# cassiePython/NeRF-Art

Measured on AMD Instinct MI355X. Metric: rays/sec at 480x270x128spp VolSDF render, higher is better.
Workload: dtype pixels bf16x3 (sdf, nabla, radiance, compositing of the 192 final samples: f32 split into 2 bf16 terms, 3 MFMAs per product, f32 accumulate), Algorithm-1 sampler fp16x1 on error-compensated one-term weights (fp16 act x fp16 weight, 1 MFMA per product, f32 accumulate; model.calibrate_sampler()), guar

## Files before the change

include/nerfart_hip.h:

```cpp
#ifndef NERFART_HIP_H
#define NERFART_HIP_H

#include <stddef.h>

#ifdef __cplusplus
extern "C" {
#endif

int nerfart_abi_version(void);
const char* nerfart_last_error(void);

int nerfart_profile_begin(void);
int nerfart_profile_end(double* ms, long long* launches, long long* units);
int nerfart_profile_end5(double* ms, long long* launches, long long* units);

void nerfart_linspace(float start, float end, int n, float* out);

int nerfart_sdf_fwd(const float* surf_blob, int precision, const float* pts, long long M, float R_bg, float* sdf_out, void* stream);
int nerfart_sdf_fwd_rays(const float* surf_blob, int precision, const float* rays_o, const float* rays_d, const int* ray_idx,
                         const float* depth, int n_slots, int n_per_ray, int depth_stride, float R_bg,
                         float* sdf_out, int out_stride, void* stream);

long long nerfart_sdf_nabla_workspace_bytes(int precision);
int nerfart_sdf_nabla_fwd(const float* surf_blob, int precision, const float* pts, long long M, float R_bg, float* sdf_out,
// ... 20 lines not shown
int nerfart_sdf_bwd2(const float* surf_blob, long long M, const float* gbar_h7, const float* gbar_sdf, void* f2_dump, void* r2_dump,
                     void* stream);

int nerfart_get_rays(const float* pose_dev, const float* K_dev, int H, int W, const long long* select_dev, int n,
                     float* rays_o, float* rays_d, void* stream);
int nerfart_normalize_dirs(const float* in, float* out, int n, void* stream);
int nerfart_linspace_depths(const float* t_dev, int n, const float* near, const float* far, float near_s, float far_s,
                            int n_rays, float* out, int stride, void* stream);

int nerfart_volsdf_first_check(int n_rays, int n, int cap, int n_final, float eps, float alpha_net, float beta_net,
                               const float* dA, const float* sA, const float* u_final, int u_final_stride,
                               float beta_plus0_denom, const float* far, float far_s, float* d_fine, float* beta_plus,
                               float* beta_map, float* iter_usage, int* act_out, int* act_count, void* stream);
int nerfart_volsdf_upsample(int n_active, int n, int cap, int n_up, const float* dA, const float* sA, const int* act,
                            const float* beta_plus, const float* u_up, int clamp_bounds, float* d_new, void* stream);
int nerfart_volsdf_merge_check(int n_active, int n, int cap, int n_up, int n_final, int max_bisect, int it, float eps,
                               float alpha_net, float beta_net, const float* dA, const float* sA, float* dB, float* sB,
                               const int* act, const float* d_new, const float* s_new, const float* u_final,
                               int u_final_stride, float* d_fine, float* beta_plus, float* beta_map, float* iter_usage,
                               int* act_out, int* act_count, void* stream);
int nerfart_volsdf_finalize(int n_active, int n, int cap, int n_final, const float* dA, const float* sA, const int* act,
                            const float* u_final, int u_final_stride, const float* beta_plus, float* d_fine,
                            float* beta_map, float* iter_usage, void* stream);
long long nerfart_volsdf_sampler_workspace_bytes(int n_rays, int n_init, int n_up, int n_final, int max_iter);
int nerfart_volsdf_fine_sample(const float* surf_blob, int precision, const float* rays_o, const float* rays_dn, int n_rays,
                               const float* near, const float* far, float near_s, float far_s, float R_bg,
                               float alpha_net, float beta_net, float eps, int n_init, int n_up, int n_final,
                               int max_iter, int max_bisect, const float* t_init_dev, const float* u_up_dev,
                               const float* u_final_dev, int u_final_per_ray, float* d_fine, float* beta_map,
                               float* iter_usage, void* workspace, long long workspace_bytes, void* stream);


int nerfart_volsdf_fine_sample_guarded(const float* surf_blob, int precision, const float* esc_blob, int esc_precision, float guard,
                                       const float* rays_o, const float* rays_dn, int n_rays,
                                       const float* near, const float* far, float near_s, float far_s, float R_bg,
                                       float alpha_net, float beta_net, float eps, int n_init, int n_up, int n_final,
                                       int max_iter, int max_bisect, const float* t_init_dev, const float* u_up_dev,
                                       const float* u_final_dev, int u_final_per_ray, float* d_fine, float* beta_map,
                                       float* iter_usage, int* n_escalated, void* workspace, long long workspace_bytes, void* stream);

int nerfart_volsdf_fine_sample_guarded2(const float* surf_blob, int precision, const float* esc_blob, int esc_precision, float guard, int late_round,
                                        const float* rays_o, const float* rays_dn, int n_rays,
                                        const float* near, const float* far, float near_s, float far_s, float R_bg,
                                        float alpha_net, float beta_net, float eps, int n_init, int n_up, int n_final,
                                        int max_iter, int max_bisect, const float* t_init_dev, const float* u_up_dev,
                                        const float* u_final_dev, int u_final_per_ray, float* d_fine, float* beta_map,
// ... 246 lines not shown
```

nerfart_amd/csrc/ray_common.h:

```cpp
#pragma once
#include "nerfart_common.h"
#include "sample_cdf.h"
#include <math.h>

namespace nerfart {

__device__ __forceinline__ float wave_sum(float v) {
#pragma unroll
    for (int o = 32; o > 0; o >>= 1) v += __shfl_xor(v, o, 64);
    return v;
}
__device__ __forceinline__ float wave_max(float v) {
#pragma unroll
    for (int o = 32; o > 0; o >>= 1) v = fmaxf(v, __shfl_xor(v, o, 64));
    return v;
}
__device__ __forceinline__ float wave_excl_sum(float v) {
    const int lane = threadIdx.x & 63;
#pragma unroll
    for (int o = 1; o < 64; o <<= 1) {
        const float t = __shfl_up(v, o, 64);
        if (lane >= o) v += t;
    }
    const float e = __shfl_up(v, 1, 64);
// ... 141 lines not shown
            const float sg = sdf_to_sigma(C.s[i], alpha, beta);
            const float t = a4b * C.dd[i];
            const float x = expf(-C.dstar[i] / beta);
            c_sigma[i] = sg; c_t[i] = t; c_x[i] = x;
            sR = __fmaf_rn(C.delta[i], sg, sR);
            sE = __fmaf_rn(t, x, sE);
        }
    }
    float R = wave_excl_sum(sR), E = wave_excl_sum(sE);
    float mx = -INFINITY;
#pragma unroll
    for (int i = 0; i < MAXSEG; ++i) {
        if (i < C.cnt) {
            E = __fmaf_rn(c_t[i], c_x[i], E);
            float b = expf(-R) * (expf(E) - 1.f);
            if (isnan(b)) b = INFINITY;
            mx = fmaxf(mx, b);
            R = __fmaf_rn(C.delta[i], c_sigma[i], R);
        }
    }
    return wave_max(mx);
}

__device__ __forceinline__ float error_bound_scan(const float* d, const float* s, int n, float alpha, float beta,
                                                  float* w_out, bool clamp) {
#ifndef NERFART_SCAN_GENERIC
    const int seg = (n - 1 + 63) >> 6;
    if (seg <= 8) return error_bound_scan_cached<8>(d, s, n, alpha, beta, w_out, clamp);
    if (seg <= 16) return error_bound_scan_cached<16>(d, s, n, alpha, beta, w_out, clamp);
    if (seg <= 24) return error_bound_scan_cached<24>(d, s, n, alpha, beta, w_out, clamp);
#endif
    return error_bound_scan_generic(d, s, n, alpha, beta, w_out, clamp);
}

__device__ __forceinline__ void opacity_cdf(const float* d, const float* s, int n, float alpha, float beta, float* cdf) {
    const int lane = threadIdx.x & 63;
    const int nint = n - 1;
    const int seg = (nint + 63) >> 6;
    const int k0 = lane * seg;
    const int k1 = (k0 + seg < nint) ? k0 + seg : nint;
    float sR = 0.f;
    for (int k = k0; k < k1; ++k) sR += sdf_to_sigma(s[k], alpha, beta) * (d[k + 1] - d[k]);
    float R = wave_excl_sum(sR);
    if (lane == 0) cdf[0] = 0.f;
    for (int k = k0; k < k1; ++k) {
        cdf[k + 1] = 1.f - expf(-R);
// ... 24 lines not shown
```

nerfart_amd/csrc/volsdf_render.hip:

```cpp
#include "ray_common.h"
#include "host_util.h"
#include <cstdlib>

namespace nerfart {

struct SamplerParams {
    int n;
    int cap;
    int n_up;
    int n_final;
    int max_bisect;
    int it;
    float eps;
    float alpha_net, beta_net;
    int u_final_stride;
    float guard;
    int* esc_list;
    int* esc_count;
};

__device__ __forceinline__ bool in_guard_band(const SamplerParams& P, float mx) {
    return P.guard > 0.f && fabsf(mx - P.eps) <= P.guard * P.eps;
}
__device__ __forceinline__ void escalate(const SamplerParams& P, int ray) {
    if (threadIdx.x == 0) P.esc_list[atomicAdd(P.esc_count, 1)] = ray;
}

__global__ void k_linspace_depths(const float* __restrict__ t, int n, const float* __restrict__ near,
                                  const float* __restrict__ far, float near_s, float far_s, int n_rays,
                                  float* __restrict__ out, int stride) {
    const long long i = (long long)blockIdx.x * blockDim.x + threadIdx.x;
    if (i >= (long long)n_rays * n) return;
    const int r = (int)(i / n), k = (int)(i - (long long)r * n);
    const float nr = near ? near[r] : near_s, fr = far ? far[r] : far_s;
    const float tk = t[k];
    out[(size_t)r * stride + k] = __fadd_rn(__fmul_rn(nr, __fsub_rn(1.f, tk)), __fmul_rn(fr, tk));
}

__global__ void k_normalize_dirs(const float* __restrict__ in, float* __restrict__ out, int n) {
    const int i = blockIdx.x * blockDim.x + threadIdx.x;
    if (i >= n) return;
// ... 68 lines not shown
}

template <int MAXSEG>
__device__ __forceinline__ void merge_check_tail(const SamplerParams& P, int ray, const float* d, const float* s, float* cdf, int nm,
                                                 const float* __restrict__ u_final, float* __restrict__ d_fine, float* __restrict__ beta_plus,
                                                 float* __restrict__ beta_map, float* __restrict__ iter_usage, int* __restrict__ act_out,
                                                 int* __restrict__ act_count) {
    constexpr int NS = MAXSEG > 0 ? MAXSEG : 1;
    SegConsts<NS> C;
    if constexpr (MAXSEG > 0) load_seg_consts<NS>(d, s, nm, C);
    auto scan = [&](float alpha, float beta) -> float {
        if constexpr (MAXSEG > 0) return scan_consts<NS>(C, alpha, beta);
        else return error_bound_scan(d, s, nm, alpha, beta, nullptr, false);
    };
    const float mx = scan(P.alpha_net, P.beta_net);
    if (in_guard_band(P, mx)) { escalate(P, ray); return; }
    if (!(mx > P.eps)) {
        opacity_cdf(d, s, nm, P.alpha_net, P.beta_net, cdf);
        __syncthreads();
        emit_final_samples(d, cdf, nm, u_final + (size_t)ray * P.u_final_stride, P.n_final, d_fine + (size_t)ray * P.n_final);
        if (threadIdx.x == 0) { iter_usage[ray] = (float)P.it; beta_map[ray] = P.beta_net; }
    } else {
        float hi = beta_plus[ray], lo = P.beta_net;
        for (int b = 0; b < P.max_bisect; ++b) {
            const float mid = 0.5f * (lo + hi);
            const float m = scan(1.f / mid, mid);
            if (m <= P.eps) hi = mid; else lo = mid;
        }
        if (threadIdx.x == 0) {
            beta_plus[ray] = hi;
            act_out[atomicAdd(act_count, 1)] = ray;
        }
    }
}

__global__ void __launch_bounds__(64)
k_merge_check(SamplerParams P, const float* __restrict__ dA, const float* __restrict__ sA,
              float* __restrict__ dB, float* __restrict__ sB, const int* __restrict__ act,
              const float* __restrict__ d_new, const float* __restrict__ s_new, const float* __restrict__ u_final,
              float* __restrict__ d_fine, float* __restrict__ beta_plus, float* __restrict__ beta_map,
              float* __restrict__ iter_usage, int* __restrict__ act_out, int* __restrict__ act_count) {
    extern __shared__ __attribute__((aligned(16))) float sm[];
    const int slot = blockIdx.x, ray = act[slot];
    const int n = P.n, nu = P.n_up, nm = n + nu;
    float* d_old = sm; float* dn = sm + n;
    float* d = dn + nu; float* s = d + nm;
    const float* s_old = sA + (size_t)ray * P.cap;
    const float* sn = s_new + (size_t)slot * nu;
    load_row(d_old, dA + (size_t)ray * P.cap, n);
    load_row(dn, d_new + (size_t)slot * nu, nu);
    __syncthreads();
    for (int i = threadIdx.x; i < n; i += 64) {
        const int r = i + lower_bound(dn, nu, d_old[i]);
        d[r] = d_old[i]; s[r] = s_old[i];
// ... 189 lines not shown
    const int first = blockIdx.x * 1024;
    int part = 0;
    for (int i = t; i < first; i += 1024) part += alive[i];
#pragma unroll
    for (int o = 32; o > 0; o >>= 1) part += __shfl_xor(part, o, 64);
    if (lane == 0) wsum[wv] = part;
    __syncthreads();
    if (t == 0) { int b = 0; for (int w = 0; w < 16; ++w) b += wsum[w]; base_sh = b; }
    __syncthreads();
    const int base = base_sh;
    const int slot = first + t;
    const bool keep = slot < n_live && alive[slot] != 0;
    const unsigned long long mask = __ballot(keep);
    const int rank = __popcll(mask & ((1ull << lane) - 1ull));
    __syncthreads();
    if (lane == 0) wsum[wv] = __popcll(mask);
    __syncthreads();
    int before = 0, total = 0;
    for (int w = 0; w < 16; ++w) { const int c = wsum[w]; if (w < wv) before += c; total += c; }
    if (keep) live_next[base + before + rank] = live[slot];
    if (t == 0 && first + 1024 >= n_live) *n_next = base + total;
}

}

using namespace nerfart;

extern "C" {

void nerfart_linspace(float start, float end, int n, float* out) {
    if (n == 1) { out[0] = start; return; }
    const float step = (end - start) / (float)(n - 1);
    const int half = n / 2;
    for (int i = 0; i < n; ++i) out[i] = (i < half) ? start + step * (float)i : end - step * (float)(n - i - 1);
}

int nerfart_normalize_dirs(const float* in, float* out, int n, void* stream) {
    if (n <= 0) return 0;
    hipLaunchKernelGGL(k_normalize_dirs, dim3((n + 255) / 256), dim3(256), 0, (hipStream_t)stream, in, out, n);
    NERFART_HIP(hipGetLastError());
    return 0;
}

int nerfart_linspace_depths(const float* t_dev, int n, const float* near, const float* far, float near_s, float far_s,
                            int n_rays, float* out, int stride, void* stream) {
    const long long tot = (long long)n_rays * n;
// ... 46 lines not shown
    if (n_up & (n_up - 1)) { set_last_error("n_up must be a power of two"); return 2; }
    SamplerParams P{n, cap, n_up, 0, 0, 0, 0.f, 0.f, 0.f};
    const size_t lds = ((size_t)4 * n + n_up) * sizeof(float);
    if (int rc = set_lds((const void*)k_upsample, lds, kLdsRefusal)) return rc;
    const char* e = std::getenv("NERFART_UPSAMPLE_SORT");
    const int always_sort = (e != nullptr && e[0] == 'a') ? 1 : 0;
    hipLaunchKernelGGL(k_upsample, dim3(n_active), dim3(64), lds, (hipStream_t)stream, P, dA, sA, act, beta_plus, u_up,
                       clamp_bounds, always_sort, d_new);
    NERFART_HIP(hipGetLastError());
    return 0;
}

int nerfart_volsdf_upsample(int n_active, int n, int cap, int n_up, const float* dA, const float* sA, const int* act,
                            const float* beta_plus, const float* u_up, int clamp_bounds, float* d_new, void* stream) {
    if (n_active <= 0) return 0;
    if (int rc = check_rows("volsdf_upsample", n, cap, 0)) return rc;
    return upsample_launch(n_active, n, cap, n_up, dA, sA, act, beta_plus, u_up, clamp_bounds, d_new, stream);
}

static int merge_check_launch(int n_active, int n, int cap, int n_up, int n_final, int max_bisect, int it, float eps,
                              float alpha_net, float beta_net, const float* dA, const float* sA, float* dB, float* sB,
                              const int* act, const float* d_new, const float* s_new, const float* u_final,
                              int u_final_stride, float* d_fine, float* beta_plus, float* beta_map, float* iter_usage,
                              int* act_out, int* act_count, float guard, int* esc_list, int* esc_count, void* stream) {
    if (n_active <= 0) return 0;
    SamplerParams P{n, cap, n_up, n_final, max_bisect, it, eps, alpha_net, beta_net, u_final_stride, guard, esc_list, esc_count};
    const size_t lds = ((size_t)3 * n + 3 * n_up) * sizeof(float);
    if (int rc = set_lds((const void*)k_merge_check, lds, kLdsRefusal)) return rc;
    hipLaunchKernelGGL(k_merge_check, dim3(n_active), dim3(64), lds, (hipStream_t)stream, P, dA, sA, dB, sB, act, d_new,
                       s_new, u_final, d_fine, beta_plus, beta_map, iter_usage, act_out, act_count);
    NERFART_HIP(hipGetLastError());
    return 0;
}

int nerfart_volsdf_merge_check(int n_active, int n, int cap, int n_up, int n_final, int max_bisect, int it, float eps,
                               float alpha_net, float beta_net, const float* dA, const float* sA, float* dB, float* sB,
                               const int* act, const float* d_new, const float* s_new, const float* u_final,
                               int u_final_stride, float* d_fine, float* beta_plus, float* beta_map, float* iter_usage,
                               int* act_out, int* act_count, void* stream) {
    if (n_active <= 0) return 0;
    if (int rc = check_rows("volsdf_merge_check", n, cap, n_up)) return rc;
    return merge_check_launch(n_active, n, cap, n_up, n_final, max_bisect, it, eps, alpha_net, beta_net, dA, sA, dB, sB, act, d_new, s_new, u_final,
                              u_final_stride, d_fine, beta_plus, beta_map, iter_usage, act_out, act_count, 0.f, nullptr, nullptr, stream);
}

static int finalize_launch(int n_active, int n, int cap, int n_final, const float* dA, const float* sA, const int* act,
                           const float* u_final, int u_final_stride, const float* beta_plus, float* d_fine,
                           float* beta_map, float* iter_usage, void* stream) {
    if (n_active <= 0) return 0;
    SamplerParams P{n, cap, 0, n_final, 0, 0, 0.f, 0.f, 0.f, u_final_stride};
    const size_t lds = (size_t)3 * n * sizeof(float);
    if (int rc = set_lds((const void*)k_finalize_unconverged, lds, kLdsRefusal)) return rc;
    hipLaunchKernelGGL(k_finalize_unconverged, dim3(n_active), dim3(64), lds, (hipStream_t)stream, P, dA, sA, act,
                       u_final, beta_plus, d_fine, beta_map, iter_usage);
    NERFART_HIP(hipGetLastError());
    return 0;
}

int nerfart_volsdf_finalize(int n_active, int n, int cap, int n_final, const float* dA, const float* sA, const int* act,
                            const float* u_final, int u_final_stride, const float* beta_plus, float* d_fine,
                            float* beta_map, float* iter_usage, void* stream) {
    if (n_active <= 0) return 0;
    if (int rc = check_rows("volsdf_finalize", n, cap, 0)) return rc;
    return finalize_launch(n_active, n, cap, n_final, dA, sA, act, u_final, u_final_stride, beta_plus, d_fine, beta_map, iter_usage, stream);
}

// ... 9 lines not shown
    return 0;
}

int nerfart_volsdf_composite(int n_rays, int P, const float* d_all, const float* sdf, const float* radiance,
                             const float* nabla, float alpha, float beta, int white_bkgd, float* rgb, float* depth,
                             float* acc, float* normals, float* sigma_out, float* p_out, float* tau_out, void* stream) {
    if (n_rays <= 0) return 0;
    if (P < 2) { set_last_error("volsdf_composite: needs P >= 2 samples per ray (P - 1 intervals)"); return 2; }
    if (normals && !nabla) { set_last_error("composite: normals requested without nablas"); return 2; }
    hipLaunchKernelGGL(k_composite_volsdf, dim3(n_rays), dim3(64), 0, (hipStream_t)stream, P, d_all, sdf, radiance, nabla,
                       alpha, beta, white_bkgd, rgb, depth, acc, normals, sigma_out, p_out, tau_out);
    NERFART_HIP(hipGetLastError());
    return 0;
}

typedef struct {
    float *dA, *sA, *dB, *sB, *d_new, *s_new, *beta_plus;
    int *act0, *act1, *count;
    float *t_init, *u_up, *u_final;
    int* esc_list;
    float *c_o, *c_dn, *c_near, *c_far, *c_u, *c_d_fine, *c_beta, *c_iter;
} sampler_ws_t;

enum { COUNT_SLOTS = 64, ESC_SLOT = COUNT_SLOTS - 1 };

static sampler_ws_t carve_sampler(Carver& c, int R, int cap, int n_up, int n0, int n_final) {
    sampler_ws_t w;
    const size_t row = (size_t)R * cap;
    w.dA = c.take<float>(row);
    w.sA = c.take<float>(row);
    w.dB = c.take<float>(row);
    w.sB = c.take<float>(row);
    w.d_new = c.take<float>((size_t)R * n_up);
    w.s_new = c.take<float>((size_t)R * n_up);
    w.beta_plus = c.take<float>((size_t)R);
    w.act0 = c.take<int>((size_t)R);
    w.act1 = c.take<int>((size_t)R);
    w.count = c.take<int>(COUNT_SLOTS);
    w.t_init = c.take<float>((size_t)n0);
    w.u_up = c.take<float>((size_t)(n_up + 2));
    w.u_final = c.take<float>((size_t)n_final);
    w.esc_list = c.take<int>((size_t)R);
    w.c_o = c.take<float>((size_t)R * 3);
    w.c_dn = c.take<float>((size_t)R * 3);
    w.c_near = c.take<float>((size_t)R);
    w.c_far = c.take<float>((size_t)R);
    w.c_u = c.take<float>((size_t)R * n_final);
// ... 3 lines not shown
    return w;
}

static size_t sampler_bytes(int R, int cap, int n_up, int n0, int n_final) {
    Carver c(nullptr);
    carve_sampler(c, R, cap, n_up, n0, n_final);
    return c.off;
}

long long nerfart_volsdf_sampler_workspace_bytes(int n_rays, int n_init, int n_up, int n_final, int max_iter) {
    return (long long)sampler_bytes(n_rays, n_init + max_iter * n_up, n_up, n_init, n_final);
}

static int fine_sample_run(const float* surf_blob, int precision, const float* esc_blob, int esc_precision, float guard, int late_round,
                           const float* rays_o, const float* rays_dn, int n_rays,
                           const float* near, const float* far, float near_s, float far_s, float R_bg,
                           float alpha_net, float beta_net, float eps, int n_init, int n_up, int n_final,
                           int max_iter, int max_bisect, const float* t_init_dev, const float* u_up_dev,
                           const float* u_final_dev, int u_final_per_ray, float* d_fine, float* beta_map,
                           float* iter_usage, void* workspace, long long workspace_bytes, int* n_escalated, hipStream_t stream) {
    if (n_escalated) *n_escalated = 0;
    if (n_rays <= 0) return 0;
    if (u_final_per_ray && !u_final_dev) { set_last_error("fine_sample: u_final_per_ray needs u_final_dev [n_rays, n_final]"); return 2; }
    if (max_iter < 0 || max_iter >= ESC_SLOT) { set_last_error("fine_sample: max_iter must be in [0, 62]"); return 2; }
    const bool guarded = esc_blob != nullptr && guard > 0.f;
    if (!guarded) guard = 0.f;
    const int u_stride = u_final_per_ray ? n_final : 0;
    const int cap = n_init + max_iter * n_up;
    Carver carver(workspace);
    sampler_ws_t w = carve_sampler(carver, n_rays, cap, n_up, n_init, n_final);
    if (!workspace || (size_t)workspace_bytes < carver.off) { set_last_error("fine_sample: workspace too small"); return 2; }
    const bool own_tables = !(t_init_dev && u_up_dev && u_final_dev);
    if (!own_tables) {
        w.t_init = const_cast<float*>(t_init_dev); w.u_up = const_cast<float*>(u_up_dev); w.u_final = const_cast<float*>(u_final_dev);
    } else {
        if (int rc = upload_linspace_tables({{w.t_init, n_init}, {w.u_up, n_up + 2}, {w.u_final, n_final}}, stream)) return rc;
        if (u_final_per_ray) w.u_final = const_cast<float*>(u_final_dev);
    }
    if (int rc = nerfart_linspace_depths(w.t_init, n_init, near, far, near_s, far_s, n_rays, w.dA, cap, stream)) return rc;
    if (int rc = nerfart_sdf_fwd_rays(surf_blob, precision, rays_o, rays_dn, nullptr, w.dA, n_rays, n_init, cap, R_bg, w.sA, cap, stream)) return rc;
    NERFART_HIP(hipMemsetAsync(w.count, 0, COUNT_SLOTS * sizeof(int), stream));
    const float denom = (float)(4.0 * (double)(n_init - 1) * log(1.0 + (double)eps));
    if (int rc = first_check_launch(n_rays, n_init, cap, n_final, eps, alpha_net, beta_net, w.dA, w.sA, w.u_final,
                                    u_stride, denom, far, far_s, d_fine, w.beta_plus, beta_map, iter_usage, w.act0,
                                    w.count, guard, w.esc_list, w.count + ESC_SLOT, stream)) return rc;
    int h_count[COUNT_SLOTS];
    NERFART_HIP(hipMemcpyAsync(h_count, w.count, sizeof(h_count), hipMemcpyDeviceToHost, stream));
    NERFART_HIP(hipStreamSynchronize(stream));
    int n_act = h_count[0];
    float *dA = w.dA, *sA = w.sA, *dB = w.dB, *sB = w.sB;
    int *act = w.act0, *act_next = w.act1;
    int n = n_init;
    for (int it = 1; it <= max_iter && n_act > 0; ++it) {
        if (int rc = upsample_launch(n_act, n, cap, n_up, dA, sA, act, w.beta_plus, w.u_up, it > 1, w.d_new, stream)) return rc;
        if (int rc = nerfart_sdf_fwd_rays(surf_blob, precision, rays_o, rays_dn, act, w.d_new, n_act, n_up, n_up, R_bg, w.s_new, n_up, stream)) return rc;
        if (int rc = merge_check_launch(n_act, n, cap, n_up, n_final, max_bisect, it, eps, alpha_net, beta_net, dA, sA,
                                        dB, sB, act, w.d_new, w.s_new, w.u_final, u_stride, d_fine, w.beta_plus,
                                        beta_map, iter_usage, act_next, w.count + it, guard, w.esc_list, w.count + ESC_SLOT, stream)) return rc;
        NERFART_HIP(hipMemcpyAsync(h_count, w.count, sizeof(h_count), hipMemcpyDeviceToHost, stream));
        NERFART_HIP(hipStreamSynchronize(stream));
        n_act = h_count[it];
        float* t;
        t = dA; dA = dB; dB = t;
        t = sA; sA = sB; sB = t;
        int* ti = act; act = act_next; act_next = ti;
        n += n_up;
        if (guarded && late_round > 0 && it >= late_round) break;
    }
    if (!guarded) {
        if (n_act > 0)
            if (int rc = finalize_launch(n_act, n, cap, n_final, dA, sA, act, w.u_final, u_stride, w.beta_plus, d_fine,
                                         beta_map, iter_usage, stream)) return rc;
        return 0;
    }
    int n_esc = h_count[ESC_SLOT];
    if (n_act > 0) {
        NERFART_HIP(hipMemcpyAsync(w.esc_list + n_esc, act, sizeof(int) * (size_t)n_act, hipMemcpyDeviceToDevice, stream));
        n_esc += n_act;
    }
    if (n_escalated) *n_escalated = n_esc;
    if (n_esc == 0) return 0;
    hipLaunchKernelGGL(k_gather_rays, dim3(n_esc), dim3(64), 0, stream, w.esc_list, n_esc, rays_o, rays_dn, near, far,
                       u_final_per_ray ? u_final_dev : (const float*)nullptr, n_final, w.c_o, w.c_dn, w.c_near, w.c_far, w.c_u);
    NERFART_HIP(hipGetLastError());
    const float* u2 = u_final_per_ray ? w.c_u : (own_tables ? nullptr : u_final_dev);
    const int* esc_list = w.esc_list;
    float *c_d_fine = w.c_d_fine, *c_beta = w.c_beta, *c_iter = w.c_iter;
    profile_class0_as(4);
    const int rc_esc = fine_sample_run(esc_blob, esc_precision, nullptr, 0, 0.f, 0, w.c_o, w.c_dn, n_esc, near ? w.c_near : nullptr, far ? w.c_far : nullptr,
                                       near_s, far_s, R_bg, alpha_net, beta_net, eps, n_init, n_up, n_final, max_iter, max_bisect,
                                       own_tables ? nullptr : t_init_dev, own_tables ? nullptr : u_up_dev, u2, u_final_per_ray, c_d_fine, c_beta, c_iter,
// ... 254 lines not shown
```

nerfart_amd/hip.py:

```python
from __future__ import annotations

import ctypes as C
import os

import torch

_HERE = os.path.dirname(os.path.abspath(__file__))
LIB_PATH = os.environ.get("NERFART_HIP_LIB", os.path.join(_HERE, "csrc", "libnerfart_hip.so"))

if not os.path.exists(LIB_PATH):
    raise ImportError(
        f"{LIB_PATH} not found: build the gfx950 kernels first "
        f"(python -c 'import __graft_entry__ as g; g.build()'  or  python -m nerfart_amd.build). "
        f"nerfart_amd has no CPU / eager-PyTorch fallback.")

lib = C.CDLL(LIB_PATH)


def csrc_sha256() -> str:
    import glob
    import hashlib
    h = hashlib.sha256()
    for f in sorted(glob.glob(os.path.join(_HERE, "csrc", "*.hip")) + glob.glob(os.path.join(_HERE, "csrc", "*.h"))
                    + glob.glob(os.path.join(_HERE, "csrc", "*.cpp"))):
# ... 11 lines not shown
    "nerfart_profile_end5": (_i, [_p, _p, _p]),
    "nerfart_sdf_fwd": (_i, [_p, _i, _p, _ll, _f, _p, _p]),
    "nerfart_sdf_fwd_rays": (_i, [_p, _i, _p, _p, _p, _p, _i, _i, _i, _f, _p, _i, _p]),
    "nerfart_sdf_nabla_workspace_bytes": (_ll, [_i]),
    "nerfart_sdf_nabla_fwd": (_i, [_p, _i, _p, _ll, _f, _p, _p, _p, _p, _ll, _p]),
    "nerfart_sdf_nabla_fwd_rays": (_i, [_p, _i, _p, _p, _p, _p, _i, _i, _i, _f, _p, _p, _p, _p, _ll, _p]),
    "nerfart_wgrad_workspace_bytes": (_ll, [_i, _ll, _i]),
    "nerfart_wgrad_bf16": (_i, [_p, _ll, _p, _ll, _i, _ll, _i, _ll, _p, _p, _i, _p, _ll, _p]),
    "nerfart_ray_points": (_i, [_p, _p, _p, _ll, _i, _p, _p, _p]),
    "nerfart_volsdf_pass2_cotangents": (_i, [_p, _p, _p, _p, _p, _p, _ll, _i, _f, _f, _ll, _p, _p, _p, _p]),
    "nerfart_wgrad_operand_embed_pair": (_i, [_p, _p, _ll, _ll, _i, _p, _p]),
    "nerfart_wgrad_operand_inputs": (_i, [_p, _i, _p, _i, _p, _ll, _ll, _p, _p]),
    "nerfart_wgrad_operand_rgb_delta": (_i, [_p, _p, _ll, _ll, _p, _p, _p, _p]),
    "nerfart_wgrad_operand_sbar_ones": (_i, [_p, _ll, _ll, _p, _p]),
    "nerfart_radiance_fwd": (_i, [_p, _i, _i, _p, _p, _ll, _p, _p, _p, _p]),
    "nerfart_radiance_fwd_rays": (_i, [_p, _i, _i, _p, _p, _p, _p, _i, _i, _i, _p, _p, _p, _p]),
    "nerfart_get_rays": (_i, [_p, _p, _i, _i, _p, _i, _p, _p, _p]),
    "nerfart_normalize_dirs": (_i, [_p, _p, _i, _p]),
    "nerfart_linspace_depths": (_i, [_p, _i, _p, _p, _f, _f, _i, _p, _i, _p]),
    "nerfart_volsdf_first_check": (_i, [_i, _i, _i, _i, _f, _f, _f, _p, _p, _p, _i, _f, _p, _f, _p, _p, _p, _p, _p, _p, _p]),
    "nerfart_volsdf_upsample": (_i, [_i, _i, _i, _i, _p, _p, _p, _p, _p, _i, _p, _p]),
    "nerfart_volsdf_merge_check": (_i, [_i, _i, _i, _i, _i, _i, _i, _f, _f, _f] + [_p] * 8 + [_i] + [_p] * 7),
    "nerfart_volsdf_finalize": (_i, [_i, _i, _i, _i] + [_p] * 4 + [_i] + [_p] * 5),
    "nerfart_volsdf_sampler_workspace_bytes": (_ll, [_i, _i, _i, _i, _i]),
    "nerfart_volsdf_fine_sample": (_i, [_p, _i, _p, _p, _i, _p, _p, _f, _f, _f, _f, _f, _f, _i, _i, _i, _i, _i, _p, _p, _p, _i, _p, _p, _p, _p, _ll, _p]),
    "nerfart_volsdf_fine_sample_guarded": (_i, [_p, _i, _p, _i, _f, _p, _p, _i, _p, _p, _f, _f, _f, _f, _f, _f, _i, _i, _i, _i, _i, _p, _p, _p, _i, _p, _p, _p, _p, _p, _ll, _p]),
    "nerfart_volsdf_fine_sample_guarded2": (_i, [_p, _i, _p, _i, _f, _i, _p, _p, _i, _p, _p, _f, _f, _f, _f, _f, _f, _i, _i, _i, _i, _i, _p, _p, _p, _i, _p, _p, _p, _p, _p, _ll, _p]),
    "nerfart_sort_concat": (_i, [_i, _p, _i, _i, _p, _i, _i, _p, _i, _p]),
    "nerfart_volsdf_composite": (_i, [_i, _i, _p, _p, _p, _p, _f, _f, _i] + [_p] * 8),
    "nerfart_volsdf_composite_bwd": (_i, [_i, _i, _p, _p, _p, _f, _f, _i, _p, _p, _p, _p, _p, _p]),
    "nerfart_neus_composite_bwd": (_i, [_i, _i, _p, _p, _f, _i, _p, _p, _p, _p, _p, _p]),
    "nerfart_volsdf_composite_geo_bwd": (_i, [_i, _i, _p, _p, _p, _f, _f, _p, _p, _p, _i, _p, _p, _p, _p]),
    "nerfart_sdf_fwd2_dump_bytes": (_ll, [_ll]),
    "nerfart_sdf_bwd2_dump_bytes": (_ll, [_ll]),
    "nerfart_sdf_fwd2": (_i, [_p, _p, _p, _ll, _p, _p]),
    "nerfart_sdf_bwd2": (_i, [_p, _ll, _p, _p, _p, _p, _p]),
    "nerfart_radiance_dump_bytes": (_ll, [_ll]),
    "nerfart_radiance_fwd_dump": (_i, [_p, _i, _p, _p, _ll, _p, _p, _p, _p, _p]),
    "nerfart_radiance_bwd": (_i, [_p, _ll, _p, _p, _p, _p, _p, _p, _p]),
    "nerfart_volsdf_render_workspace_bytes": (_ll, [_i, _i, _i, _i, _i]),
    "nerfart_volsdf_render_fwd": (_i, [_p, _p, _i, _i, _p, _p, _i, _f, _f, _f, _f, _f, _f, _i, _i, _i, _i, _i, _i] + [_p] * 4 + [_i] + [_p] * 13 + [_p, _ll, _p]),
    "nerfart_volsdf_render_mixed_fwd": (_i, [_p, _p, _i, _p, _i, _i, _p, _p, _i, _f, _f, _f, _f, _f, _f, _i, _i, _i, _i, _i, _i] + [_p] * 4 + [_i] + [_p] * 13 + [_p, _ll, _p]),
    "nerfart_volsdf_render_staged_fwd": (_i, [_p, _i, _p, _i, _p, _i, _f, _i, _p, _p, _i, _f, _f, _f, _f, _f, _f, _i, _i, _i, _i, _i, _i] + [_p] * 4 + [_i] + [_p] * 13 + [_p, _p, _ll, _p]),
    "nerfart_volsdf_render_staged2_fwd": (_i, [_p, _i, _p, _i, _p, _i, _f, _i, _i, _p, _p, _i, _f, _f, _f, _f, _f, _f, _i, _i, _i, _i, _i, _i] + [_p] * 4 + [_i] + [_p] * 13 + [_p, _p, _ll, _p]),
    "nerfart_near_far_from_sphere": (_i, [_p, _p, _i, _f, _p, _p, _p]),
    "nerfart_neus_upsample_step": (_i, [_i, _i, _i, _i, _f, _p, _p, _p, _i, _p, _p]),
# ... 703 lines not shown
    key = (n, str(device))
    if key not in _lin_cache:
        _lin_cache[key] = torch.linspace(0, 1, n).float().to(device)
    return _lin_cache[key]


_ws_cache = {}
_ws_lock = __import__("threading").Lock()


def _workspace(nbytes: int, device) -> torch.Tensor:
    key = (str(device), int(torch.cuda.current_stream(device).cuda_stream))
    with _ws_lock:
        ws = _ws_cache.get(key)
        if ws is None or ws.numel() < nbytes:
            _ws_cache.pop(key, None)
            while len(_ws_cache) >= 8:
                _ws_cache.pop(next(iter(_ws_cache)), None)
            ws = torch.empty(int(nbytes), dtype=torch.uint8, device=device)
            _ws_cache[key] = ws
    return ws


def volsdf_fine_sample(surf_blob, rays_o, rays_dn, near: float, far: float, R_bg: float, alpha: float, beta: float,
                       eps: float, n_init: int, n_up: int, n_final: int, max_iter: int, max_bisect: int, precision: int = 0,
                       u_final=None, escalate=None, guard: float = 0.0, stats=None, late_round: int = 0):
    R = rays_o.shape[0]
    dev = rays_o.device
    if u_final is not None and tuple(u_final.shape) != (R, n_final):
        raise ValueError(f"u_final must be [{R}, {n_final}]")
    d_fine = torch.empty(R, n_final, dtype=torch.float32, device=dev)
    beta_map = torch.empty(R, dtype=torch.float32, device=dev)
    usage = torch.empty(R, dtype=torch.float32, device=dev)
    nb = lib.nerfart_volsdf_sampler_workspace_bytes(R, n_init, n_up, n_final, max_iter)
    ws = _workspace(nb, dev)
    esc_blob, esc_prec = escalate if (escalate is not None and guard > 0) else (None, 0)
    n_esc = C.c_int(0)
    _check(lib.nerfart_volsdf_fine_sample_guarded2(_dev(surf_blob), int(precision), _dev(esc_blob, name="esc_blob"), int(esc_prec), float(guard), int(late_round),
                                                  _dev(rays_o), _dev(rays_dn), R, None, None, float(near), float(far),
                                                  float(R_bg), float(alpha), float(beta), float(eps), n_init, n_up, n_final, max_iter,
                                                  max_bisect, _dev(lin_table(n_init, dev)), _dev(lin_table(n_up + 2, dev)),
                                                  _dev(lin_table(n_final, dev) if u_final is None else u_final, name="u_final"),
                                                  int(u_final is not None), _dev(d_fine), _dev(beta_map), _dev(usage), C.byref(n_esc), ws.data_ptr(),
                                                  ws.numel(), _stream()), "nerfart_volsdf_fine_sample_guarded2")
    if stats is not None:
        stats["escalated"] = stats.get("escalated", 0) + n_esc.value
        stats["rays"] = stats.get("rays", 0) + R
    return d_fine, beta_map, usage


def sdf_fwd2(surf_blob, pts, direction):
    M = pts.shape[0]
    dump = torch.empty(int(lib.nerfart_sdf_fwd2_dump_bytes(M)), dtype=torch.uint8, device=pts.device)
    _check(lib.nerfart_sdf_fwd2(_dev(surf_blob), _dev(pts, name="pts"), _dev(direction, name="direction"), M, dump.data_ptr(), _stream()),
           "nerfart_sdf_fwd2")
    return dump


def sdf_bwd2(surf_blob, gbar_h7, gbar_sdf, f2_dump):
    M = gbar_sdf.shape[0]
    dump = torch.empty(int(lib.nerfart_sdf_bwd2_dump_bytes(M)), dtype=torch.uint8, device=gbar_sdf.device)
    _check(lib.nerfart_sdf_bwd2(_dev(surf_blob), M, _dev(gbar_h7, name="gbar_h7"), _dev(gbar_sdf, name="gbar_sdf"), f2_dump.data_ptr(),
                                dump.data_ptr(), _stream()), "nerfart_sdf_bwd2")
    return dump


def radiance_fwd_dump(rad_blob, view_tiles: int, pts, view, nabla, h7):
    M = pts.shape[0]
    rgb = torch.empty(M, 3, dtype=torch.float32, device=pts.device)
    dump = torch.empty(int(lib.nerfart_radiance_dump_bytes(M)), dtype=torch.uint8, device=pts.device)
# ... 173 lines not shown
def volsdf_render(surf_blob, rad_blob, view_tiles, rays_o, rays_d, *, near, far, R_bg, alpha, beta, eps=0.1,
                  n_samples=128, n_importance=64, max_upsample_steps=5, max_bisection_steps=10, white_bkgd=False,
                  calc_normal=True, detailed=False, k3_rays_chunk=8192, precision=0, u_final=None, sampler=None, guard: float = 0.0,
                  radiance=None, stats=None, late_round: int = 0):
    R = rays_o.shape[0]
    dev = rays_o.device
    P = n_samples + n_importance
    if u_final is not None and tuple(u_final.shape) != (R, n_importance):
        raise ValueError(f"u_final must be [{R}, {n_importance}]")
    f = lambda *s: torch.empty(*s, dtype=torch.float32, device=dev)
    out = {"rgb": f(R, 3), "depth_volume": f(R), "mask_volume": f(R)}
    if calc_normal:
        out["normals_volume"] = f(R, 3)
    det = {}
    if detailed:
        det = {"d_vals": f(R, P), "implicit_surface": f(R, P), "implicit_nablas": f(R, P, 3), "radiance": f(R, P, 3),
               "sigma": f(R, P), "p_i": f(R, P - 1), "visibility_weights": f(R, P - 1), "beta_map": f(R), "iter_usage": f(R)}
    nb = lib.nerfart_volsdf_render_workspace_bytes(R, n_samples, n_importance, max_upsample_steps, k3_rays_chunk)
    ws = _workspace(nb, dev)
    g = lambda k: _dev(det.get(k))
    samp_blob, samp_prec = sampler if sampler is not None else (surf_blob, precision)
    rblob, rprec = radiance if radiance is not None else (rad_blob, precision)
    n_esc = C.c_int(0)
    _check(lib.nerfart_volsdf_render_staged2_fwd(
        _dev(surf_blob), int(precision), _dev(rblob, name="rad_blob"), int(rprec), _dev(samp_blob, name="sampler_blob"), int(samp_prec), float(guard),
        int(late_round), int(view_tiles), _dev(rays_o, name="rays_o"), _dev(rays_d, name="rays_d"), R,
        float(near), float(far), float(R_bg), float(alpha), float(beta), float(eps), n_samples, n_importance,
        max_upsample_steps, max_bisection_steps, int(bool(white_bkgd)), k3_rays_chunk,
        _dev(lin_table(n_samples, dev)), _dev(lin_table(4 * n_samples, dev)), _dev(lin_table(4 * n_samples + 2, dev)),
        _dev(lin_table(n_importance, dev) if u_final is None else u_final, name="u_final"), int(u_final is not None),
        _dev(out["rgb"]), _dev(out["depth_volume"]), _dev(out["mask_volume"]), _dev(out.get("normals_volume")),
        g("d_vals"), g("implicit_surface"), g("implicit_nablas"), g("radiance"), g("sigma"), g("p_i"),
        g("visibility_weights"), g("beta_map"), g("iter_usage"), C.byref(n_esc), ws.data_ptr(), ws.numel(), _stream()),
        "nerfart_volsdf_render_staged2_fwd")
    if stats is not None:
        stats["escalated"] = stats.get("escalated", 0) + n_esc.value
        stats["rays"] = stats.get("rays", 0) + R
    out.update(det)
    return out


def volsdf_render_mixed(surf_blob, rad_blob, sampler_blob, sampler_precision: int, view_tiles, rays_o, rays_d, *, near, far, R_bg, alpha, beta, eps=0.1,
                        n_samples=128, n_importance=64, max_upsample_steps=5, max_bisection_steps=10, white_bkgd=False, calc_normal=True,
                        detailed=False, k3_rays_chunk=8192, precision=1, u_final=None, guard: float = 0.0, late_round: int = 0):
    R = rays_o.shape[0]
    dev = rays_o.device
    P = n_samples + n_importance
    f = lambda *s: torch.empty(*s, dtype=torch.float32, device=dev)
    dn = normalize_dirs(rays_d)
    d_fine, beta_map, usage = volsdf_fine_sample(sampler_blob, rays_o, dn, near, far, R_bg, alpha, beta, eps, 4 * n_samples, 4 * n_samples, n_importance,
                                                 max_upsample_steps, max_bisection_steps, precision=sampler_precision, u_final=u_final,
                                                 escalate=(surf_blob, precision), guard=guard, late_round=late_round)
    d_coarse = f(R, n_samples)
    _check(lib.nerfart_linspace_depths(_dev(lin_table(n_samples, dev)), n_samples, None, None, float(near), float(far), R, _dev(d_coarse), n_samples,
                                       _stream()), "nerfart_linspace_depths")
    d_all = f(R, P)
    _check(lib.nerfart_sort_concat(R, _dev(d_coarse), n_samples, n_samples, _dev(d_fine), n_importance, n_importance, _dev(d_all), P, _stream()),
           "nerfart_sort_concat")
    sdf, nab, rad = f(R, P), f(R, P, 3), f(R, P, 3)
    ws, nb = nabla_workspace(precision, dev)
# ... 118 lines not shown
```

Baseline: 341,000.

## Decide bisection scan predicate with a fast bounded exp2 check and exact fallback

Inside the beta bisection of the VolSDF merge-check kernel, each midpoint now runs a cheaper scan built on exp2 intrinsics, with conservative error margins that can certify the bound is at most eps or above it. When the margins cannot decide, or inputs fall outside safe ranges, it falls back to the exact scan. This is meant to cut transcendental cost in the bisection loop. It also adds device atomic counters for scans and fallbacks, an env var to force the exact path, and a predicate test kernel, all of which add some overhead and risk of decision mismatches near the threshold.

After: 341,900, median of 6. No clear change (+0.3%).

```diff
diff --git a/include/nerfart_hip.h b/include/nerfart_hip.h
--- a/include/nerfart_hip.h
+++ b/include/nerfart_hip.h
@@ -66,6 +66,10 @@
 int nerfart_volsdf_finalize(int n_active, int n, int cap, int n_final, const float* dA, const float* sA, const int* act,
                             const float* u_final, int u_final_stride, const float* beta_plus, float* d_fine,
                             float* beta_map, float* iter_usage, void* stream);
+void nerfart_volsdf_scan_counts(long long* scans, long long* fallbacks);
+int nerfart_volsdf_scan_predicate_test(int n_rows, int n, const float* d, const float* s, int n_beta, const float* betas, float eps,
+                                       const float* eps_each, int variant, int* bits, float* mx_exact, float* b_fast, float* r_fast,
+                                       float* e_fast, float* b_exact, void* stream);
 long long nerfart_volsdf_sampler_workspace_bytes(int n_rays, int n_init, int n_up, int n_final, int max_iter);
 int nerfart_volsdf_fine_sample(const float* surf_blob, int precision, const float* rays_o, const float* rays_dn, int n_rays,
                                const float* near, const float* far, float near_s, float far_s, float R_bg,
diff --git a/nerfart_amd/csrc/ray_common.h b/nerfart_amd/csrc/ray_common.h
--- a/nerfart_amd/csrc/ray_common.h
+++ b/nerfart_amd/csrc/ray_common.h
@@ -187,6 +187,72 @@
     return wave_max(mx);
 }
 
+constexpr float SCAN_KAPPA = 0x1p-15f;
+constexpr float SCAN_ABS = 0x1p-18f;
+constexpr float SCAN_DEC_SLACK = 1.0625f;
+constexpr float SCAN_R_CLAMP = 64.f;
+constexpr float SCAN_E_MAX = 40.f;
+constexpr float SCAN_LOG2E = 1.44269504088896341f;
+
+struct ScanLeRow { float ek, c_lo, c_hi; bool ok; };
+
+template <int MAXSEG>
+__device__ __forceinline__ ScanLeRow scan_le_row(const SegConsts<MAXSEG>& C, float eps, float kappa = SCAN_KAPPA, float abs_term = SCAN_ABS) {
+    bool bad = false;
+#pragma unroll
+    for (int i = 0; i < MAXSEG; ++i)
+        if (i < C.cnt) bad |= !(fabsf(C.s[i]) <= 0x1p20f) | !(C.dstar[i] <= 0x1p20f) | !(C.delta[i] >= 0.f) | !(C.delta[i] <= 0x1p8f);
+    ScanLeRow G;
+    G.ok = !__any((int)bad) && eps >= 0x1p-10f && eps <= 0x1p10f;
+    G.ek = eps * (kappa * SCAN_DEC_SLACK);
+    G.c_lo = eps - abs_term * SCAN_DEC_SLACK - G.ek;
+    G.c_hi = eps + abs_term * SCAN_DEC_SLACK + G.ek;
+    return G;
+}
+
+template <int MAXSEG>
+__device__ __forceinline__ int scan_consts_fast(const SegConsts<MAXSEG>& C, const ScanLeRow& G, float alpha, float beta,
+                                                float* bf_out = nullptr, float* r_out = nullptr, float* e_out = nullptr, int k0 = 0) {
+    if (!(G.ok && alpha >= 0x1p-14f && alpha <= 0x1p14f && beta >= 0x1p-14f && beta <= 0x1p6f)) return 0;
+    const float a4b = alpha / (4.f * beta);
+    const float c = -SCAN_LOG2E / beta;
+    float c_sigma[MAXSEG], c_q[MAXSEG];
+    float sR = 0.f, sE = 0.f;
+#pragma unroll
+    for (int i = 0; i < MAXSEG; ++i) {
+        const float e = __builtin_amdgcn_exp2f(__fmaf_rn(fabsf(C.s[i]), c, -1.f));
+        const float sg = alpha * ((C.s[i] >= 0.f) ? e : 1.f - e);
+        const float q = (a4b * C.dd[i]) * __builtin_amdgcn_exp2f(C.dstar[i] * c);
+        c_sigma[i] = sg; c_q[i] = q;
+        sR = __fmaf_rn(C.delta[i], sg, sR);
+        sE += q;
+    }
+    float R = wave_excl_sum(sR), E = wave_excl_sum(sE);
+    bool le = true, gt = false;
+#pragma unroll
+    for (int i = 0; i < MAXSEG; ++i) {
+        E += c_q[i];
+        const float Rc = fminf(R, SCAN_R_CLAMP);
+        const float bf = __builtin_amdgcn_exp2f(Rc * -SCAN_LOG2E) * (__builtin_amdgcn_exp2f(E * SCAN_LOG2E) - 1.f);
+        const float re = Rc + E;
+        const bool pad = i >= C.cnt;
+        le = le && ((bf <= __fmaf_rn(-G.ek, re, G.c_lo)) || pad);
+        gt = gt || ((bf > __fmaf_rn(G.ek, re, G.c_hi)) && !pad);
+        if (bf_out && !pad) { bf_out[k0 + i] = bf; r_out[k0 + i] = Rc; e_out[k0 + i] = E; }
+        R = __fmaf_rn(C.delta[i], c_sigma[i], R);
+    }
+    if (!(E <= SCAN_E_MAX)) { le = false; gt = false; }
+    if (__any((int)gt)) return 2;
+    return __all((int)le) ? 1 : 0;
+}
+
+template <int MAXSEG>
+__device__ __forceinline__ bool scan_consts_le(const SegConsts<MAXSEG>& C, float alpha, float beta, float eps, bool* undecided = nullptr) {
+    const int dec = scan_consts_fast<MAXSEG>(C, scan_le_row<MAXSEG>(C, eps), alpha, beta);
+    if (undecided) *undecided = dec == 0;
+    return dec == 0 ? scan_consts<MAXSEG>(C, alpha, beta) <= eps : dec == 1;
+}
+
 __device__ __forceinline__ float error_bound_scan(const float* d, const float* s, int n, float alpha, float beta,
                                                   float* w_out, bool clamp) {
 #ifndef NERFART_SCAN_GENERIC
diff --git a/nerfart_amd/csrc/volsdf_render.hip b/nerfart_amd/csrc/volsdf_render.hip
--- a/nerfart_amd/csrc/volsdf_render.hip
+++ b/nerfart_amd/csrc/volsdf_render.hip
@@ -1,5 +1,6 @@
 #include "ray_common.h"
 #include "host_util.h"
+#include <atomic>
 #include <cstdlib>
 
 namespace nerfart {
@@ -17,6 +18,8 @@
     float guard;
     int* esc_list;
     int* esc_count;
+    int scan_exact;
+    int* scan_count;
 };
 
 __device__ __forceinline__ bool in_guard_band(const SamplerParams& P, float mx) {
@@ -131,14 +134,25 @@
         if (threadIdx.x == 0) { iter_usage[ray] = (float)P.it; beta_map[ray] = P.beta_net; }
     } else {
         float hi = beta_plus[ray], lo = P.beta_net;
+        int n_fallback = 0;
+#ifdef NERFART_SCAN_EXACT
+        const bool fast = false;
+#else
+        const bool fast = MAXSEG > 0 && !P.scan_exact;
+#endif
+        ScanLeRow G{};
+        if constexpr (MAXSEG > 0) { if (fast) G = scan_le_row<NS>(C, P.eps); }
         for (int b = 0; b < P.max_bisect; ++b) {
             const float mid = 0.5f * (lo + hi);
-            const float m = scan(1.f / mid, mid);
-            if (m <= P.eps) hi = mid; else lo = mid;
+            int dec = 0;
+            if constexpr (MAXSEG > 0) { if (fast) dec = scan_consts_fast<NS>(C, G, 1.f / mid, mid); }
+            if (dec == 0) { dec = scan(1.f / mid, mid) <= P.eps ? 1 : 2; n_fallback += fast ? 1 : 0; }
+            if (dec == 1) hi = mid; else lo = mid;
         }
         if (threadIdx.x == 0) {
             beta_plus[ray] = hi;
             act_out[atomicAdd(act_count, 1)] = ray;
+            if (P.scan_count) { atomicAdd(P.scan_count, P.max_bisect); atomicAdd(P.scan_count + 1, n_fallback); }
         }
     }
 }
@@ -374,6 +388,41 @@
     if (t == 0 && first + 1024 >= n_live) *n_next = base + total;
 }
 
+template <int MAXSEG>
+__device__ __forceinline__ void scan_predicate_test_tail(const float* d, const float* s, int n, float beta, float eps, int variant, int* bits,
+                                                         float* mx_exact, float* b_fast, float* r_fast, float* e_fast, float* b_exact) {
+    SegConsts<MAXSEG> C;
+    load_seg_consts<MAXSEG>(d, s, n, C);
+    const float alpha = 1.f / beta;
+    const int seg = (n - 1 + 63) >> 6, k0 = (threadIdx.x & 63) * seg;
+    const ScanLeRow G = scan_le_row<MAXSEG>(C, eps, variant == 1 ? 0.5f * SCAN_KAPPA : SCAN_KAPPA, variant == 2 ? 0.f : SCAN_ABS);
+    const int dec = scan_consts_fast<MAXSEG>(C, G, alpha, beta, b_fast, r_fast, e_fast, k0);
+    const float mx = scan_consts<MAXSEG>(C, alpha, beta);
+    bool und = dec == 0;
+    bool le = und ? mx <= eps : dec == 1;
+    if (variant == 0) le = scan_consts_le<MAXSEG>(C, alpha, beta, eps, &und);
+    if (b_exact) error_bound_scan_cached<MAXSEG>(d, s, n, alpha, beta, b_exact, false);
+    if (threadIdx.x == 0) { *bits = (le ? 1 : 0) | (mx <= eps ? 2 : 0) | (und ? 4 : 0); *mx_exact = mx; }
+}
+
+__global__ void __launch_bounds__(64)
+k_scan_predicate_test(int n, const float* __restrict__ dA, const float* __restrict__ sA, int n_beta, const float* __restrict__ betas, float eps,
+                      const float* __restrict__ eps_each, int variant, int* __restrict__ bits, float* __restrict__ mx_exact,
+                      float* __restrict__ b_fast, float* __restrict__ r_fast, float* __restrict__ e_fast, float* __restrict__ b_exact) {
+    extern __shared__ __attribute__((aligned(16))) float sm[];
+    const int row = blockIdx.x, j = blockIdx.y;
+    const size_t q = (size_t)row * n_beta + j, qi = q * (size_t)(n - 1);
+    float* d = sm; float* s = sm + n;
+    load_row(d, dA + (size_t)row * n, n);
+    load_row(s, sA + (size_t)row * n, n);
+    __syncthreads();
+    const float e = eps_each ? eps_each[q] : eps;
+    float* bf = b_fast ? b_fast + qi : nullptr; float* rf = b_fast ? r_fast + qi : nullptr; float* ef = b_fast ? e_fast + qi : nullptr;
+    float* be = b_exact ? b_exact + qi : nullptr;
+    if (((n - 1 + 63) >> 6) <= 16) scan_predicate_test_tail<16>(d, s, n, betas[q], e, variant, bits + q, mx_exact + q, bf, rf, ef, be);
+    else scan_predicate_test_tail<24>(d, s, n, betas[q], e, variant, bits + q, mx_exact + q, bf, rf, ef, be);
+}
+
 }
 
 using namespace nerfart;
@@ -466,9 +515,11 @@
                               float alpha_net, float beta_net, const float* dA, const float* sA, float* dB, float* sB,
                               const int* act, const float* d_new, const float* s_new, const float* u_final,
                               int u_final_stride, float* d_fine, float* beta_plus, float* beta_map, float* iter_usage,
-                              int* act_out, int* act_count, float guard, int* esc_list, int* esc_count, void* stream) {
+                              int* act_out, int* act_count, float guard, int* esc_list, int* esc_count, int* scan_count, void* stream) {
     if (n_active <= 0) return 0;
-    SamplerParams P{n, cap, n_up, n_final, max_bisect, it, eps, alpha_net, beta_net, u_final_stride, guard, esc_list, esc_count};
+    const char* e = std::getenv("NERFART_SCAN_EXACT");
+    const int scan_exact = (e != nullptr && e[0] != '\0' && e[0] != '0') ? 1 : 0;
+    SamplerParams P{n, cap, n_up, n_final, max_bisect, it, eps, alpha_net, beta_net, u_final_stride, guard, esc_list, esc_count, scan_exact, scan_count};
     const size_t lds = ((size_t)3 * n + 3 * n_up) * sizeof(float);
     if (int rc = set_lds((const void*)k_merge_check, lds, kLdsRefusal)) return rc;
     hipLaunchKernelGGL(k_merge_check, dim3(n_active), dim3(64), lds, (hipStream_t)stream, P, dA, sA, dB, sB, act, d_new,
@@ -485,7 +536,24 @@
     if (n_active <= 0) return 0;
     if (int rc = check_rows("volsdf_merge_check", n, cap, n_up)) return rc;
     return merge_check_launch(n_active, n, cap, n_up, n_final, max_bisect, it, eps, alpha_net, beta_net, dA, sA, dB, sB, act, d_new, s_new, u_final,
-                              u_final_stride, d_fine, beta_plus, beta_map, iter_usage, act_out, act_count, 0.f, nullptr, nullptr, stream);
+                              u_final_stride, d_fine, beta_plus, beta_map, iter_usage, act_out, act_count, 0.f, nullptr, nullptr, nullptr, stream);
+}
+
+int nerfart_volsdf_scan_predicate_test(int n_rows, int n, const float* d, const float* s, int n_beta, const float* betas, float eps,
+                                       const float* eps_each, int variant, int* bits, float* mx_exact, float* b_fast, float* r_fast,
+                                       float* e_fast, float* b_exact, void* stream) {
+    if (n_rows <= 0 || n_beta <= 0) return 0;
+    if (n < 2 || n > 24 * 64 + 1) { set_last_error("volsdf_scan_predicate_test: needs 2 <= n <= 1537 (segments of at most 24 intervals per lane)"); return 2; }
+    if (n_beta > 65535) { set_last_error("volsdf_scan_predicate_test: n_beta must be at most 65535"); return 2; }
+    if (variant < 0 || variant > 2) { set_last_error("volsdf_scan_predicate_test: variant must be 0, 1 or 2"); return 2; }
+    if (!d || !s || !betas || !bits || !mx_exact) { set_last_error("volsdf_scan_predicate_test: d, s, betas, bits or mx_exact is NULL"); return 2; }
+    if ((b_fast == nullptr) != (r_fast == nullptr) || (b_fast == nullptr) != (e_fast == nullptr)) {
+        set_last_error("volsdf_scan_predicate_test: b_fast, r_fast and e_fast go together"); return 2;
+    }
+    hipLaunchKernelGGL(k_scan_predicate_test, dim3(n_rows, n_beta), dim3(64), (size_t)2 * n * sizeof(float), (hipStream_t)stream, n, d, s, n_beta,
+                       betas, eps, eps_each, variant, bits, mx_exact, b_fast, r_fast, e_fast, b_exact);
+    NERFART_HIP(hipGetLastError());
+    return 0;
 }
 
 static int finalize_launch(int n_active, int n, int cap, int n_final, const float* dA, const float* sA, const int* act,
@@ -541,7 +609,14 @@
     float *c_o, *c_dn, *c_near, *c_far, *c_u, *c_d_fine, *c_beta, *c_iter;
 } sampler_ws_t;
 
-enum { COUNT_SLOTS = 64, ESC_SLOT = COUNT_SLOTS - 1 };
+enum { COUNT_SLOTS = 64, ESC_SLOT = COUNT_SLOTS - 1, SCAN_SLOT = COUNT_SLOTS - 3 };
+
+static std::atomic<long long> g_scan_total{0}, g_scan_fallback{0};
+
+void nerfart_volsdf_scan_counts(long long* scans, long long* fallbacks) {
+    if (scans) *scans = g_scan_total.load();
+    if (fallbacks) *fallbacks = g_scan_fallback.load();
+}
 
 static sampler_ws_t carve_sampler(Carver& c, int R, int cap, int n_up, int n0, int n_final) {
     sampler_ws_t w;
@@ -591,7 +666,7 @@
     if (n_escalated) *n_escalated = 0;
     if (n_rays <= 0) return 0;
     if (u_final_per_ray && !u_final_dev) { set_last_error("fine_sample: u_final_per_ray needs u_final_dev [n_rays, n_final]"); return 2; }
-    if (max_iter < 0 || max_iter >= ESC_SLOT) { set_last_error("fine_sample: max_iter must be in [0, 62]"); return 2; }
+    if (max_iter < 0 || max_iter >= SCAN_SLOT) { set_last_error("fine_sample: max_iter must be in [0, 60]"); return 2; }
     const bool guarded = esc_blob != nullptr && guard > 0.f;
     if (!guarded) guard = 0.f;
     const int u_stride = u_final_per_ray ? n_final : 0;
@@ -625,7 +700,7 @@
         if (int rc = nerfart_sdf_fwd_rays(surf_blob, precision, rays_o, rays_dn, act, w.d_new, n_act, n_up, n_up, R_bg, w.s_new, n_up, stream)) return rc;
         if (int rc = merge_check_launch(n_act, n, cap, n_up, n_final, max_bisect, it, eps, alpha_net, beta_net, dA, sA,
                                         dB, sB, act, w.d_new, w.s_new, w.u_final, u_stride, d_fine, w.beta_plus,
-                                        beta_map, iter_usage, act_next, w.count + it, guard, w.esc_list, w.count + ESC_SLOT, stream)) return rc;
+                                        beta_map, iter_usage, act_next, w.count + it, guard, w.esc_list, w.count + ESC_SLOT, w.count + SCAN_SLOT, stream)) return rc;
         NERFART_HIP(hipMemcpyAsync(h_count, w.count, sizeof(h_count), hipMemcpyDeviceToHost, stream));
         NERFART_HIP(hipStreamSynchronize(stream));
         n_act = h_count[it];
@@ -636,6 +711,8 @@
         n += n_up;
         if (guarded && late_round > 0 && it >= late_round) break;
     }
+    g_scan_total += h_count[SCAN_SLOT];
+    g_scan_fallback += h_count[SCAN_SLOT + 1];
     if (!guarded) {
         if (n_act > 0)
             if (int rc = finalize_launch(n_act, n, cap, n_final, dA, sA, act, w.u_final, u_stride, w.beta_plus, d_fine,
diff --git a/nerfart_amd/hip.py b/nerfart_amd/hip.py
--- a/nerfart_amd/hip.py
+++ b/nerfart_amd/hip.py
@@ -57,6 +57,8 @@
     "nerfart_volsdf_upsample": (_i, [_i, _i, _i, _i, _p, _p, _p, _p, _p, _i, _p, _p]),
     "nerfart_volsdf_merge_check": (_i, [_i, _i, _i, _i, _i, _i, _i, _f, _f, _f] + [_p] * 8 + [_i] + [_p] * 7),
     "nerfart_volsdf_finalize": (_i, [_i, _i, _i, _i] + [_p] * 4 + [_i] + [_p] * 5),
+    "nerfart_volsdf_scan_counts": (None, [_p, _p]),
+    "nerfart_volsdf_scan_predicate_test": (_i, [_i, _i, _p, _p, _i, _p, _f, _p, _i, _p, _p, _p, _p, _p, _p, _p]),
     "nerfart_volsdf_sampler_workspace_bytes": (_ll, [_i, _i, _i, _i, _i]),
     "nerfart_volsdf_fine_sample": (_i, [_p, _i, _p, _p, _i, _p, _p, _f, _f, _f, _f, _f, _f, _i, _i, _i, _i, _i, _p, _p, _p, _i, _p, _p, _p, _p, _ll, _p]),
     "nerfart_volsdf_fine_sample_guarded": (_i, [_p, _i, _p, _i, _f, _p, _p, _i, _p, _p, _f, _f, _f, _f, _f, _f, _i, _i, _i, _i, _i, _p, _p, _p, _i, _p, _p, _p, _p, _p, _ll, _p]),
@@ -806,6 +808,38 @@
     return ws
 
 
+def scan_counts():
+    a, b = C.c_longlong(0), C.c_longlong(0)
+    lib.nerfart_volsdf_scan_counts(C.cast(C.byref(a), C.c_void_p), C.cast(C.byref(b), C.c_void_p))
+    return a.value, b.value
+
+
+def _add_sampler_stats(stats, R, n_esc, scans0):
+    scans1 = scan_counts()
+    stats["escalated"] = stats.get("escalated", 0) + n_esc
+    stats["rays"] = stats.get("rays", 0) + R
+    stats["bisect_scans"] = stats.get("bisect_scans", 0) + scans1[0] - scans0[0]
+    stats["bisect_fallbacks"] = stats.get("bisect_fallbacks", 0) + scans1[1] - scans0[1]
+
+
+def scan_predicate_test(d, s, betas, eps=0.1, eps_each=None, variant=0, dumps=False):
+    rows, n = d.shape
+    nb = betas.shape[1]
+    dev = d.device
+    bits = torch.zeros(rows, nb, dtype=torch.int32, device=dev)
+    mx = torch.empty(rows, nb, dtype=torch.float32, device=dev)
+    bf = rf = ef = be = None
+    if dumps:
+        bf, rf, ef, be = (torch.full((rows, nb, n - 1), float("nan"), dtype=torch.float32, device=dev) for _ in range(4))
+    _check(lib.nerfart_volsdf_scan_predicate_test(rows, n, _dev(d, name="d"), _dev(s, name="s"), nb, _dev(betas, name="betas"), float(eps),
+                                                  _dev(eps_each, name="eps_each"), int(variant), _dev(bits, torch.int32), _dev(mx), _dev(bf), _dev(rf),
+                                                  _dev(ef), _dev(be), _stream()), "nerfart_volsdf_scan_predicate_test")
+    out = {"le": (bits & 1) != 0, "le_exact": (bits & 2) != 0, "undecided": (bits & 4) != 0, "mx_exact": mx}
+    if dumps:
+        out.update(b_fast=bf, r_fast=rf, e_fast=ef, b_exact=be)
+    return out
+
+
 def volsdf_fine_sample(surf_blob, rays_o, rays_dn, near: float, far: float, R_bg: float, alpha: float, beta: float,
                        eps: float, n_init: int, n_up: int, n_final: int, max_iter: int, max_bisect: int, precision: int = 0,
                        u_final=None, escalate=None, guard: float = 0.0, stats=None, late_round: int = 0):
@@ -820,6 +854,7 @@
     ws = _workspace(nb, dev)
     esc_blob, esc_prec = escalate if (escalate is not None and guard > 0) else (None, 0)
     n_esc = C.c_int(0)
+    scans0 = scan_counts()
     _check(lib.nerfart_volsdf_fine_sample_guarded2(_dev(surf_blob), int(precision), _dev(esc_blob, name="esc_blob"), int(esc_prec), float(guard), int(late_round),
                                                   _dev(rays_o), _dev(rays_dn), R, None, None, float(near), float(far),
                                                   float(R_bg), float(alpha), float(beta), float(eps), n_init, n_up, n_final, max_iter,
@@ -828,8 +863,7 @@
                                                   int(u_final is not None), _dev(d_fine), _dev(beta_map), _dev(usage), C.byref(n_esc), ws.data_ptr(),
                                                   ws.numel(), _stream()), "nerfart_volsdf_fine_sample_guarded2")
     if stats is not None:
-        stats["escalated"] = stats.get("escalated", 0) + n_esc.value
-        stats["rays"] = stats.get("rays", 0) + R
+        _add_sampler_stats(stats, R, n_esc.value, scans0)
     return d_fine, beta_map, usage
 
 
@@ -1049,6 +1083,7 @@
     samp_blob, samp_prec = sampler if sampler is not None else (surf_blob, precision)
     rblob, rprec = radiance if radiance is not None else (rad_blob, precision)
     n_esc = C.c_int(0)
+    scans0 = scan_counts()
     _check(lib.nerfart_volsdf_render_staged2_fwd(
         _dev(surf_blob), int(precision), _dev(rblob, name="rad_blob"), int(rprec), _dev(samp_blob, name="sampler_blob"), int(samp_prec), float(guard),
         int(late_round), int(view_tiles), _dev(rays_o, name="rays_o"), _dev(rays_d, name="rays_d"), R,
@@ -1061,8 +1096,7 @@
         g("visibility_weights"), g("beta_map"), g("iter_usage"), C.byref(n_esc), ws.data_ptr(), ws.numel(), _stream()),
         "nerfart_volsdf_render_staged2_fwd")
     if stats is not None:
-        stats["escalated"] = stats.get("escalated", 0) + n_esc.value
-        stats["rays"] = stats.get("rays", 0) + R
+        _add_sampler_stats(stats, R, n_esc.value, scans0)
     out.update(det)
     return out
 
```
